# AllenInstitute/distributed-vae

Measured on AMD Instinct MI355X. Metric: cells/sec per train step (fwd+loss+bwd+opt), higher is better.
Workload: dtype f32; 1 GPU; cpl_mixVAE A=2 arms, synthetic-10x-v1 50000 cells x 5000 genes per GPU, batch 5000/GPU, fp32, H=100 L=10 C=92 S=2, x_drop=0.5, Adam lr=1e-3; global_batch=5000, parallelism=dp1, noise=in-kernel Philox4x32-10

## Files before the change

### distributed-vae_amd/_native.py

```python
from __future__ import annotations

import ctypes as C
import os
from typing import Dict, Optional

import torch

HERE = os.path.dirname(os.path.abspath(__file__))
LIB_PATH = os.environ.get("MMVAE_LIB") or os.path.join(HERE, "libmmvae_hip.so")

ABI_VERSION = 5
N_PARAM_TENSORS = 28
N_BN = 6
MAX_ARMS = 8

PARAM_NAMES = [
    "fc1.weight", "fc1.bias", "fc2.weight", "fc2.bias", "fc3.weight", "fc3.bias", "fc4.weight", "fc4.bias",
    "fc5.weight", "fc5.bias", "fcc.weight", "fcc.bias", "fc_mu.weight", "fc_sigma.weight", "fc_mu.bias",
    "fc_sigma.bias", "fc6.weight", "fc6.bias", "fc7.weight", "fc7.bias", "fc8.weight", "fc8.bias",
    "fc9.weight", "fc9.bias", "fc10.weight", "fc10.bias", "fc11.weight", "fc11.bias",
]
BN_NAMES = ["batch_l1", "batch_l2", "batch_l3", "batch_l4", "batch_l5", "batch_s"]

WS_IDS = {name: i for i, name in enumerate([
# ... 89 lines not shown
    out = (C.c_int32 * PLAN_FIELDS)()
    check(lib().mmvae_debug_plan(C.byref(dims), C.byref(hyper), C.byref(ex) if ex is not None else None, CALL_KINDS[kind],
                                 int(params_align), int(x_align), int(x_arm_stride), int(bool(has_x16)), int(bool(fc11_grad)),
                                 C.byref(out)), "mmvae_debug_plan")
    plan = {}
    for name, v in zip(PLAN_NAMES, out):
        if name in PLAN_ENUMS:
            plan[name] = PLAN_ENUMS[name][v]
        elif name == "kind":
            plan[name] = next(k for k, i in CALL_KINDS.items() if i == v)
        elif name in ("gd10_slabs", "dw11_slabs"):
            plan[name] = int(v)
        else:
            plan[name] = bool(v)
    return plan


_lib = None


def lib():
    global _lib
    if _lib is not None:
        return _lib
    if not os.path.exists(LIB_PATH):
        raise NativeError(
            f"{LIB_PATH} not found: build the HIP extension first "
            "(python -c 'import __graft_entry__ as g; g.build()' or python distributed-vae_amd/build.py). "
            "There is no CPU fallback.")
    L = C.CDLL(LIB_PATH)
# ... 15 lines not shown
                                 C.c_size_t, vp, ex, vp]
    L.mmvae_adam_step.argtypes = [i64, vp, vp, vp, vp, i64, f32, f32, f32, f32, f32, i32, vp]
    L.mmvae_train_step.argtypes = [C.POINTER(Dims), C.POINTER(Hyper), C.POINTER(Noise), vp, vp, vp, vp, i64, vp,
                                   C.c_size_t, vp, vp, i32, vp, vp, i64, f32, f32, f32, f32, f32, i32, ex, vp]
    L.mmvae_train_step_rows.argtypes = [C.POINTER(Dims), C.POINTER(Hyper), C.POINTER(Noise), vp, vp, vp, vp, vp, i64, i64, vp, vp,
                                        C.c_size_t, vp, vp, i32, vp, vp, i64, f32, f32, f32, f32, f32, i32, ex, vp]
    L.mmvae_train_step_rows.restype = C.c_int
    L.mmvae_to_bf16.argtypes = [vp, i64, i64, i32, vp, vp]
    L.mmvae_to_bf16.restype = C.c_int
    L.mmvae_debug_stage.argtypes = [C.POINTER(Dims), C.POINTER(Hyper), C.POINTER(Noise), i32, vp, vp, i64, vp,
                                    C.c_size_t, vp, ex, vp]
    L.mmvae_dump_noise.argtypes = [C.POINTER(Dims), C.POINTER(Hyper), C.POINTER(Noise), vp, vp, vp, vp, vp]
    L.mmvae_debug_plan.argtypes = [C.POINTER(Dims), C.POINTER(Hyper), ex, i32, i32, i32, i64, i32, i32,
                                   C.POINTER(C.c_int32 * PLAN_FIELDS)]
    L.mmvae_debug_plan.restype = C.c_int
    L.mmvae_eval_classify.argtypes = [C.POINTER(Dims), C.POINTER(Hyper), vp, vp, vp, i64, vp, C.c_size_t, vp, vp, ex,
                                      vp]
    L.mmvae_classify.argtypes = [vp, i64, i32, vp, vp]
    L.mmvae_confmat_accumulate.argtypes = [vp, i32, i64, i32, vp, vp]
    L.mmvae_consensus.argtypes = [vp, i32, i32, vp, vp, vp]
    L.mmvae_aug_packed_floats.argtypes = [C.POINTER(AugDims)]
    L.mmvae_aug_packed_floats.restype = C.c_size_t
    L.mmvae_aug_workspace_bytes.argtypes = [C.POINTER(AugDims), i32]
    L.mmvae_aug_workspace_bytes.restype = C.c_size_t
    L.mmvae_aug_pack.argtypes = [C.POINTER(AugDims), C.POINTER(AugTensors), vp, vp]
    L.mmvae_augment.argtypes = [C.POINTER(AugDims), vp, vp, i64, vp, vp, f32, vp, C.c_size_t, vp, vp, i32, ex, vp]
    L.mmvae_gather_rows.argtypes = [vp, i64, i64, vp, i64, i32, vp, vp]
    L.mmvae_tp_planes_bytes.argtypes = [i64, i32, i32]
    L.mmvae_tp_planes_bytes.restype = C.c_size_t
    L.mmvae_tp_planes.argtypes = [vp, i64, i64, i32, i32, vp, vp]
# ... 338 lines not shown
```

### distributed-vae_amd/csrc/api.hip

```cpp
#include "common.hpp"
#include <stdarg.h>
#include <stdio.h>
#include <string.h>

namespace mmvae {

static thread_local char g_err[512] = "";
void set_error(const char* fmt, ...) {
    va_list ap;
    va_start(ap, fmt);
    vsnprintf(g_err, sizeof(g_err), fmt, ap);
    va_end(ap);
}

Splits default_splits(const mmvae_dims& d, const mmvae_exec* ex) {
    int g_split[6] = {0, 0, 0, 0, 0, 0};
    if (ex) for (int i = 0; i < 6; ++i) g_split[i] = ex->split[i] > 0 && ex->split[i] <= 64 ? ex->split[i] : 0;
    constexpr int CUS = 256;
    auto fit = [](int base_blocks, int slots, int cap) {
        const int base = base_blocks > 0 ? base_blocks : 1;
        auto eff = [&](int k) { const int n = base * k; return (double)n / (double)(((n + slots - 1) / slots) * slots); };
        int pick = 1;
        double best = 0.0;
        for (int k = 1; k <= cap; ++k) {
            if (eff(k) >= 0.93) { pick = k; break; }
            if (eff(k) > best + 1e-9) { best = eff(k); pick = k; }
        }
        for (int k = pick + 1; k <= cap && k <= pick + 2; ++k)
            if (eff(k) >= 0.995) return k;
// ... 35 lines not shown
        if (g_split[5] <= 0) {
            const int nwg = max(1, pairs_d * d.A);
            const bool chain_x3 = chain_planes_fit(d) && !ex->tune[MMVAE_TUNE_CHAIN_FP32];
            const int target = chain_x3 ? 140 : 3 * CUS / 8;
            s.ks_dw11 = min(max(1, (target + nwg / 2) / nwg), max(1, cdiv(d.B, 32)));
        }
        if (g_split[3] <= 0) s.ks_small = min(fit(cdiv(N_SMALL * d.A, 2), CUS, 32), max(1, cdiv(d.B, 32)));
    }
    if (ex && ex->tune[MMVAE_TUNE_ENGINE] == 1 && fastdims && bf16_tiles_fit(d)) {
        if (g_split[3] <= 0) s.ks_small = min(fit(cdiv(N_SMALL * d.A, 2), CUS, 32), max(1, cdiv(d.B, 32)));
        if (g_split[5] <= 0) {
            const int nwg = max(1, cdiv(d.D, 128) * d.A);
            s.ks_dw11 = min(max(1, (5 * CUS / 8 + nwg / 2) / nwg), max(1, cdiv(d.B, 32)));
        }
    }
    return s;
}

POff make_poff(const mmvae_dims& d) {
    POff p{};
    const int64_t D = d.D, H = d.H, L = d.L, C = d.C, S = d.S;
    const int64_t sizes[MMVAE_N_PARAM_TENSORS] = {
        H * D, H, H * H, H, H * H, H, H * H, H, L * H, L, C * L, C, S * (L + C), S * (L + C), S, S,
        L * (C + S), L, H * L, H, H * H, H, H * H, H, H * H, H, D * H, D};
    int64_t off = 0;
    for (int t = 0; t < MMVAE_N_PARAM_TENSORS; ++t) {
        if (t != 13 && t != 15) off = cdiv64(off, 4) * 4;
        p.o[t] = off;
        off += sizes[t];
    }
// ... 41 lines not shown
    L.acc_end = off;
    L.GD10_slab = take((int64_t)max(L.sp.ns_fc11, L.sp.ks_gd10) * A * B * H);
    L.DZ11 = take(A * B * D);
    L.couple_part = take(nb * 2);
    L.T_part = take(nb * A * C); L.T = take(A * C);
    for (int i = 1; i <= 10; ++i) L.DZ[i] = take(A * B * ((i == 5 || i == 6) ? Ld : H));
    L.GZIN = take(A * B * (C + S)); L.GMS = take(A * B * 2 * S); L.GZC = take(A * B * C);
    for (int i = 1; i <= 5; ++i) {
        const int64_t W = (i == 5) ? Ld : H;
        L.G[i] = take(A * B * W);
        L.bnb_part[i] = take(A * (i == 5 ? (nb > cdiv(B, LAT_ROWS_BWD) ? nb : (int64_t)cdiv(B, LAT_ROWS_BWD)) : nb) * 2 * W);
        L.bnb_sum[i] = take(A * 2 * W);
    }
    L.dw1_slab = take((int64_t)L.sp.ks_dw * A * H * D);
    L.dw11_slab = take((int64_t)max(L.sp.ks_dw, L.sp.ks_dw11) * A * D * DW11_LD);
    L.small_slab = take((int64_t)L.sp.ks_small * A * N_SMALL * NP * SMALL_LD);
    L.xbits = take(A * B * cdiv(d.D, 32));
    {
        const int64_t Dk = cdiv64(D, 32) * 32, Dr = cdiv64(D, 128) * 128, Br = cdiv64(B, 256) * 256;
        L.pl_w1 = take(A * 3 * 128 * Dk / 2);
        L.pl_w11 = take(A * 3 * Dr * 128 / 2);
        L.pl_dz1 = take(A * 3 * Br * 128 / 2);
        L.pl_d10 = take(A * 3 * Br * 128 / 2);
        L.pl_small = take(A * (int64_t)PL_SMALL_SLOTS * 3 * 128 * 128 / 2);
    }
    L.rowmap = take(B + MAP_PAD);
    L.total = off;
    return L;
}

static int check_dims(const mmvae_dims* d) {
// ... 95 lines not shown
    else if (fc11_grad && d.H == 100 && (int64_t)cdiv(d.B, 256) * L.sp.ks_gd10 <= L.n11) p.fc11 = FC11_ZG;
    else p.fc11 = FC11_ZT;
    p.gd10_slabs = p.fast ? L.sp.ks_gd10 : L.sp.ns_fc11;
    p.dw11_slabs = p.fast ? L.sp.ks_dw11 : L.sp.ks_dw;
    p.chain_planes = p.fast && bf16_tiles && chain_planes_fit(d) && !c.tune(MMVAE_TUNE_CHAIN_FP32);
    p.lat_half = d.C <= 32 * LH_CPL && d.L <= 32 && 2 * d.S <= 32;
    p.narrow = h.gemm_bf16 == 1 && c.x16 != nullptr && bf16_tiles_fit(d) && (d.D & 7) == 0;
    p.presplit = fwd && p.fast && (x3 || p.chain_planes);
    p.bwd_small_planes = kind == CALL_BACKWARD && p.chain_planes;
    p.d10_planes = x3;
    p.dz1_in_apply = (x3 || p.narrow) && (d.H & 1) == 0;
    if (fwd && h.training) p.zero = p.presplit && dropout ? ZERO_PRESPLIT : p.fast && dropout ? ZERO_XBITS : ZERO_MEMSET;
    p.rowmap = kind == CALL_STEP_ROWS && p.zero == ZERO_PRESPLIT && slots && (p.fc11 == FC11_X3 || p.fc11 == FC11_BF16);
    p.dz11_bf16 = p.rowmap && c.x16 != nullptr && p.fc11 == FC11_BF16;
    p.dw11_side = (step || kind == CALL_BACKWARD) && p.fast && side;
    p.loss_on_side = step && p.fast && side;
    const int cs = c.tune(MMVAE_TUNE_COUPLE_SIDE);
    const bool role = p.loss_on_side && c.use_acc() && p.chain_planes && d.A >= 2 && d.A <= 5 && cs != 1 && (d.A >= 4 || cs == 3);
    p.couple = step && side ? (role ? COUPLE_IN_DEC : COUPLE_SIDE) : COUPLE_INLINE;
    p.lat_fork_rides = p.couple == COUPLE_SIDE && p.lat_half;
    p.fc11_fork_rides = p.loss_on_side && (p.fc11 == FC11_X3 || p.fc11 == FC11_BF16);
    if (kind == CALL_DECODE) {
        if (!p.fast) p.fc11 = FC11_GENERAL;
        else if (p.big == GEMM_X3 && x3_fc11_fits(d)) p.fc11 = FC11_OUT_X3;
        else if (p.big == GEMM_BF16) p.fc11 = FC11_OUT_BF16;
        else p.fc11 = FC11_ZT;
        p.d10_planes = p.fc11 == FC11_OUT_X3 || p.fc11 == FC11_OUT_BF16;
        p.dec_planes = p.d10_planes || p.chain_planes;
    }
}
// ... 95 lines not shown
static int do_loss(const Ctx& c, float* loss_out) {
    int rc;
    if ((rc = launch_couple(c))) return rc;
    return launch_loss_finalize(c, loss_out);
}

static int do_backward(const Ctx& c, const mmvae_noise* nz, const float* params, const float* x, int64_t xs,
                       float grad_scale, float* grads, const AdamHost* adam = nullptr, float* loss_out = nullptr) {
    const Plan& p = c.plan;
    int rc;
    const bool early = p.dw11_side && !adam && c.ex.early_grad_event != nullptr;
    const bool side_red = p.dw11_side && adam;
    if (c.ex_out) c.ex_out->early_recorded = 0;
    Ctx cs = c;
    cs.stream = c.side();
    if (p.dw11_side) {
        if ((rc = fork_to_side(c, EV_FORK, p.fc11_fork_rides))) return rc;
        if ((rc = dw11(cs))) return rc;
        if (early) {
            if ((rc = launch_reduce_grads(cs, grads, grad_scale, nullptr, 1))) return rc;
            if (hipEventRecord(reinterpret_cast<hipEvent_t>(c.ex.early_grad_event), c.side()) != hipSuccess) {
                set_error("event record failed");
                return MMVAE_E_LAUNCH;
            }
            if (c.ex_out) c.ex_out->early_recorded = 1;
        }
        if (side_red) {
            if ((rc = launch_reduce_grads(cs, grads, grad_scale, adam, 1))) return rc;
        }
        if (p.loss_on_side && (rc = launch_loss_finalize(cs, loss_out, 2))) return rc;
        if ((rc = record_on_side(c, EV_JOIN))) return rc;
    }
    if (p.bwd_small_planes && (rc = launch_x3_planes(c, params, false))) return rc;
    if ((rc = launch_chain_bwd_dec(c, params))) return rc;
    if (p.loss_on_side && p.couple == COUPLE_SIDE && (rc = join_from_side(c, EV_COUPLE))) return rc;
    if ((rc = launch_lat_bwd(c, nz, params))) return rc;
    for (int layer = 5; layer >= 2; --layer)
        if ((rc = launch_chain_bwd_enc(c, layer, params))) return rc;
    if ((rc = launch_bn_bwd_apply1(c))) return rc;
    if (p.big == GEMM_GENERAL) {
        if ((rc = launch_dw_big(c, nz, x, xs))) return rc;
    } else {
        if ((rc = dw1(c, x, xs))) return rc;
        if (!p.dw11_side && (rc = dw11(c))) return rc;
    }
    if ((rc = launch_dw_small(c))) return rc;
    if (p.dw11_side && (rc = join_from_side(c, EV_JOIN))) return rc;
    return launch_reduce_grads(c, grads, grad_scale, adam, early || side_red ? 2 : 3);
}

}

using namespace mmvae;

extern "C" {

int mmvae_abi_version(void) { return 5; }
const char* mmvae_last_error_string(void) { return g_err; }
int mmvae_check_dims(const mmvae_dims* d) { return check_dims(d); }

int mmvae_param_layout(const mmvae_dims* d, mmvae_param_layout_t* out) {
// ... 310 lines not shown
            if (stage == 10) return fc11_main(c, params, x, x_arm_stride, nullptr, 1);
            if (stage == 11) return fc11_gd10(c, params, nullptr, 1);
            if (stage == 12) return dw1(c, x, x_arm_stride);
            if (stage == 13) return dw11(c);
            return fc1_gemm(c, params, x, x_arm_stride);
        case 3: return launch_dw_small(c);
        case 4: return launch_chain_fwd_dec(c, params);
        case 5: return launch_chain_bwd_dec(c, params);
        case 6: return launch_lat_fwd(c, nz, params, nullptr, nullptr);
        case 7: return launch_lat_bwd(c, nz, params);
        case 8: if (!grads) { set_error("grads is null"); return MMVAE_E_BADARG; } return launch_reduce_grads(c, grads, 1.f, nullptr);
        default: set_error("unknown stage %d", stage); return MMVAE_E_BADARG;
    }
}

int mmvae_debug_plan(const mmvae_dims* d, const mmvae_hyper* h, const mmvae_exec* ex, int call_kind, int params_align,
                     int x_align, int64_t x_arm_stride, int has_x16, int fc11_grad, int32_t out[MMVAE_PLAN_FIELDS]) {
    if (int rc = check_dims(d)) return rc;
    if (!h || !out) { set_error("null hyper / out"); return MMVAE_E_BADARG; }
    if (int rc = check_gemm_engine(h->gemm_bf16)) return rc;
    static_assert(MMVAE_CALL_STEP == CALL_STEP && MMVAE_CALL_STEP_ROWS == CALL_STEP_ROWS && MMVAE_CALL_FORWARD == CALL_FORWARD &&
                  MMVAE_CALL_BACKWARD == CALL_BACKWARD && MMVAE_CALL_LOSS == CALL_LOSS && MMVAE_CALL_CLASSIFY == CALL_CLASSIFY &&
                  MMVAE_CALL_REPLAY == CALL_REPLAY && MMVAE_CALL_DECODE == CALL_DECODE && MMVAE_CALL_TRAVERSE == CALL_TRAVERSE,
                  "MMVAE_CALL_* (include/mmvae.h) are the values of CallKind");
    if (call_kind < CALL_STEP || call_kind > CALL_TRAVERSE) { set_error("unknown call kind %d", call_kind); return MMVAE_E_BADARG; }
    if (params_align < 0 || x_align < 0) { set_error("negative alignment"); return MMVAE_E_BADARG; }
    Ctx c{};
    c.d = *d;
    c.h = *h;
    if (call_kind == CALL_DECODE || call_kind == CALL_TRAVERSE || call_kind == CALL_CLASSIFY) c.h.training = 0;
    if (ex) c.ex = *ex; else memset(&c.ex, 0, sizeof(c.ex));
    c.lay = make_layout(*d, &c.ex);
    c.po = make_poff(*d);
    const uintptr_t base = 1u << 20;
    const float* params = reinterpret_cast<const float*>(base + (uintptr_t)(params_align & 15));
    const float* x = reinterpret_cast<const float*>(2 * base + (uintptr_t)(x_align & 15));
    if (has_x16 && call_kind == CALL_STEP_ROWS) c.x16 = reinterpret_cast<const unsigned short*>(3 * base);
    make_plan(c, (CallKind)call_kind, params, x, x_arm_stride, fc11_grad != 0);
    const Plan& p = c.plan;
    const int32_t v[] = {(int32_t)p.kind, p.fast, (int32_t)p.big, p.small_x3, (int32_t)p.fc11, p.gd10_slabs, p.dw11_slabs, p.chain_planes,
                         p.lat_half, p.narrow, p.presplit, p.bwd_small_planes, p.d10_planes, p.dz1_in_apply, p.dec_planes,
                         (int32_t)p.zero, p.rowmap, p.dz11_bf16, p.dw11_side, p.loss_on_side, (int32_t)p.couple, p.lat_fork_rides,
                         p.fc11_fork_rides};
    static_assert(sizeof(v) / sizeof(v[0]) == MMVAE_PLAN_FIELDS, "one value per field of Plan, in declaration order");
    for (int i = 0; i < MMVAE_PLAN_FIELDS; ++i) out[i] = v[i];
    return 0;
}

int mmvae_dump_noise(const mmvae_dims* d, const mmvae_hyper* h, const mmvae_noise* nz, uint8_t* x_mask,
                     float* u_gumbel, float* u_state, uint8_t* s_mask, void* stream) {
    if (int rc = check_dims(d)) return rc;
    if (!h || !nz) { set_error("null hyper / noise"); return MMVAE_E_BADARG; }
    return launch_dump_noise(*d, *h, nz, x_mask, u_gumbel, u_state, s_mask, reinterpret_cast<hipStream_t>(stream));
}

}
```

### distributed-vae_amd/csrc/common.hpp

```cpp
#pragma once
#include <hip/hip_runtime.h>
#include <hip/hip_ext.h>
#include <stdint.h>
#include "../../include/mmvae.h"
#include "tune.h"

namespace mmvae {

typedef float f32x16 __attribute__((ext_vector_type(16)));

constexpr int WAVE = 64;
constexpr int ROWS32 = 32;
constexpr int NP = 128;
constexpr int MAP_PAD = 256;
constexpr int DW11_LD = 132;
constexpr int SMALL_LD = 256;

__host__ __device__ inline int cdiv(int a, int b) { return (a + b - 1) / b; }
__host__ __device__ inline int64_t cdiv64(int64_t a, int64_t b) { return (a + b - 1) / b; }
__host__ __device__ inline int rup(int a, int b) { return cdiv(a, b) * b; }
__host__ __device__ inline int64_t imin64(int64_t a, int64_t b) { return a < b ? a : b; }

struct Splits {
    int ks_fc1;
    int ns_fc11;
    int ks_dw;
    int ks_dw11;
    int ks_small;
    int ks_gd10;
};

constexpr int N_SMALL = 12;

struct Layout {
    int nblk32;
    int nblk64;
    Splits sp;
    int64_t R[5];
    int nblkc;
    int chain_rows_fwd, nblkf;
    int nblkl;
    int64_t bn_mean[5], bn_rstd[5];
    int64_t bn_part[5];
    int64_t XLOW, CPROB, CC, YSOFT, CSMP, Y, MS, MU, LV, SS, ZIN;
    int64_t Dk[5];
    int64_t c_part, c_mean, c_iv;
    int64_t lat_part;
    int64_t fc1_slab;
    int n11;
    int64_t fc11_part;
    int64_t GD10_slab;
    int64_t DZ11;
    int64_t couple_part;
    int64_t T_part, T;
    int64_t DZ[11];
    int64_t GZIN, GMS, GZC, G[6];
    int64_t bnb_part[6], bnb_sum[6];
    int64_t dw1_slab;
    int64_t dw11_slab;
    int64_t small_slab;
    int64_t xbits;
    int64_t pl_w1;
    int64_t pl_w11;
    int64_t pl_dz1;
    int64_t pl_d10;
    int64_t pl_small;
    int64_t acc;
    int64_t acc_end;
    int64_t rowmap;
    int64_t total;
};
constexpr int PL_SMALL_LAYERS = 9, PL_SMALL_DEC0 = 4, PL_SMALL_SLOTS = 2 * PL_SMALL_LAYERS;
constexpr int ACC_W = 128;
constexpr int ACC_SET_I64 = 6 * ACC_W + 8;
constexpr int ACC_SET_FLOATS = 2 * ACC_SET_I64;
// ... 530 lines not shown
                const u32x4 r = xmask_words(nz, arm, (uint32_t)row, (uint32_t)(w * ncall + j));
                for (int e = 0; e < epc; ++e) word |= xmask_field_keep(nz, r, (uint32_t)e) ? (1u << (j * epc + e)) : 0u;
            }
            const int left = D - 32 * w;
            if (left < 32) word &= (1u << left) - 1u;
            out[w] = word;
        }
    }
}
#endif

inline bool fast_dims(const mmvae_dims& d) { return (d.D & 3) == 0 && (d.H & 3) == 0; }
inline bool bf16_tiles_fit(const mmvae_dims& d) { return d.H <= 124; }
inline bool x3_fc11_fits(const mmvae_dims& d) { return d.H + 1 <= 112; }
inline bool chain_planes_fit(const mmvae_dims& d) { return d.C + d.S <= 128 && d.L <= 128; }
inline bool fc11_slots_fit(const Layout& L, int B) { return (int64_t)cdiv(B, 128) * L.sp.ks_gd10 <= L.n11; }

enum CallKind { CALL_STEP, CALL_STEP_ROWS, CALL_FORWARD, CALL_BACKWARD, CALL_LOSS, CALL_CLASSIFY, CALL_REPLAY ,
                CALL_DECODE , CALL_TRAVERSE  };
enum GemmFamily { GEMM_GENERAL, GEMM_FP32, GEMM_BF16, GEMM_X3 };
enum Fc11Family { FC11_GENERAL, FC11_ZG, FC11_ZT, FC11_BF16, FC11_X3, FC11_OUT_BF16, FC11_OUT_X3 };
enum FwdZero { ZERO_NONE, ZERO_MEMSET, ZERO_XBITS , ZERO_PRESPLIT  };
enum CouplePlace { COUPLE_INLINE, COUPLE_SIDE, COUPLE_IN_DEC };
struct Plan {
    CallKind kind;
    bool fast;
    GemmFamily big;
    bool small_x3;
    Fc11Family fc11;
    int gd10_slabs;
// ... 2 lines not shown
    bool lat_half;
    bool narrow;
    bool presplit;
    bool bwd_small_planes;
    bool d10_planes;
    bool dz1_in_apply;
    bool dec_planes;
    FwdZero zero;
    bool rowmap;
    bool dz11_bf16;
    bool dw11_side;
    bool loss_on_side;
    CouplePlace couple;
    bool lat_fork_rides;
    bool fc11_fork_rides;
};

struct Ctx {
    mmvae_dims d;
    mmvae_hyper h;
    Layout lay;
    POff po;
    float* ws;
    hipStream_t stream;
    mmvae_exec ex;
    mmvae_exec* ex_out;
    hipStream_t side() const { return reinterpret_cast<hipStream_t>(ex.side_stream); }
    hipEvent_t ev(int i) const { return reinterpret_cast<hipEvent_t>(ex.ev[i]); }
    int tune(int i) const { return ex.tune[i]; }
    bool use_acc() const { return !ex.tune[MMVAE_TUNE_BN_PARTIALS]; }
// ... 7 lines not shown
    Plan plan{};
};
inline int zero_fc11_part(const Ctx& c) {
    if (c.plan.zero != ZERO_NONE) return 0;
    hipError_t e = hipMemsetAsync(c.ws + c.lay.fc11_part, 0, sizeof(float) * 2 * (size_t)c.d.A * c.lay.n11, c.stream);
    if (e != hipSuccess) { set_error("memset: %s", hipGetErrorString(e)); return MMVAE_E_LAUNCH; }
    return 0;
}
#ifdef __HIPCC__
template <class K, class... Args>
inline void launch_k(const Ctx& c, hipEvent_t stop_ev, K kernel, dim3 grid, dim3 block, unsigned shm, Args... args) {
    if (stop_ev) hipExtLaunchKernelGGL(kernel, grid, block, shm, c.stream, nullptr, stop_ev, 0, args...);
    else hipLaunchKernelGGL(kernel, grid, block, shm, c.stream, args...);
}
#endif
enum { EV_LAT = 0, EV_COUPLE, EV_FC11, EV_FORK, EV_JOIN, EV_DEC, EV_ENC, EV_SPARE  };

#ifdef __HIPCC__
NoiseDev make_noise_dev(const mmvae_noise* nz, const mmvae_hyper& h);
#endif

int launch_fc1_fwd(const Ctx& c, const mmvae_noise* nz, const float* params, const float* x, int64_t xs);
int launch_bn_eval_stats(const Ctx& c, const float* bn_running);
int launch_chain_fwd_enc(const Ctx& c, int layer , const float* params, float* bn_running, int64_t* nbt);
int launch_chain_fwd_enc_eval(const Ctx& c, const float* params);
int launch_lat_fwd(const Ctx& c, const mmvae_noise* nz, const float* params, float* bn_running, int64_t* nbt,
                   int32_t* labels = nullptr );
int launch_chain_fwd_dec(const Ctx& c, const float* params);
int launch_fc11_fused(const Ctx& c, const float* params, const float* x, int64_t xs, float* x_rec, int need_grad);
int launch_couple(const Ctx& c);
int launch_loss_finalize(const Ctx& c, float* loss_out, int mode = 0 );
// ... 2 lines not shown
int launch_chain_bwd_enc(const Ctx& c, int layer , const float* params);
int launch_bn_bwd_apply1(const Ctx& c);
int launch_dw_big(const Ctx& c, const mmvae_noise* nz, const float* x, int64_t xs);
int launch_dw_small(const Ctx& c, int which = 3 );
struct TnDesc {
    const float* P; int64_t p_arm_stride; int ldp; int Mv;
    const float* Q; int64_t q_arm_stride; int ldq; int Nv;
    int q_ones;
    int q_xmask;
    const float* q_mean;
    const float* q_rstd;
    float* out; int64_t out_arm_stride; int64_t out_ks_stride; int ldo;
};

struct TnDescs { TnDesc d[N_SMALL]; };
int launch_dw_small_x3(const Ctx& c, const TnDescs& ts, int nsel);
struct AdamHost { float* p; float* m; float* v; int64_t step; float lr, b1, b2, eps, wd; int decoupled; };
int launch_reduce_grads(const Ctx& c, float* grads, float grad_scale, const AdamHost* adam,
                        int which = 3 );
int launch_adam(int64_t n, float* p, const float* g, float* m, float* v, int64_t step, float lr, float b1,
                float b2, float eps, float wd, int decoupled, hipStream_t s);
int launch_make_xbits(const Ctx& c, const mmvae_noise* nz);
int launch_forward_zero(const Ctx& c, const mmvae_noise* nz);
int launch_fc1_epi(const Ctx& c, const float* params);
int launch_fc1_fwd_fp32(const Ctx& c, const float* params, const float* x, int64_t xs);
int launch_fc11_zg(const Ctx& c, const float* params, const float* x, int64_t xs, float* x_rec, int need_grad);
int launch_fc11_zt(const Ctx& c, const float* params, const float* x, int64_t xs, float* x_rec, int need_grad);
int launch_gd10_fp32(const Ctx& c, const float* params);
int launch_dw1_fp32(const Ctx& c, const float* x, int64_t xs);
int launch_dw11_fp32(const Ctx& c);
int launch_x3_planes(const Ctx& c, const float* params, bool head, const mmvae_noise* nz = nullptr);
// ... 44 lines not shown
```

### distributed-vae_amd/csrc/gemm_bf16.hip

```cpp
#include "common.hpp"

namespace mmvae {

typedef __bf16 bf16x8 __attribute__((ext_vector_type(8)));
typedef __bf16 bf16x2 __attribute__((ext_vector_type(2)));
typedef unsigned int u32x4v __attribute__((ext_vector_type(4)));


constexpr int BT = 128;
constexpr int KT = 64;
constexpr int LDB = 36;
constexpr int LDK = 136;

template <int NP>
struct Eng {
    static constexpr int KT = NP == 1 ? 64 : 32;
    static constexpr int NQ = KT / 8;
    static constexpr int LDB = KT / 2 + 4;
    static constexpr int PLANE = BT * LDB;
    static constexpr int LDK = NP == 1 ? 136 : 160;
    static constexpr int NBUF = NP == 1 ? 2 : 1;
};

__device__ __forceinline__ unsigned pack_bf16(float a, float b) {
// ... 1689 lines not shown

int launch_dw11_bf16(const Ctx& c) {
    const mmvae_dims& d = c.d;
    const Layout& L = c.lay;
    GemmArgs g{};
    g.a = kminor(c.ws + L.DZ11, d.D, d.D, d.B); g.a_arm = (int64_t)d.B * d.D;
    g.b = kminor(c.ws + L.Dk[4], d.H, d.H, d.B); g.b_arm = (int64_t)d.B * d.H;
    g.b.ones_row = d.H;
    if (c.plan.big == GEMM_X3) use_planes(c, g.b, PL_D10);
    else if (c.plan.dz11_bf16) { g.a.src16 = 1; g.a_arm /= 2; }
    g.M = d.D; g.N = d.H + 1; g.K = d.B; g.KS = L.sp.ks_dw11; g.A = d.A;
    g.so = SlabOut{c.ws + L.dw11_slab, (int64_t)d.A * d.D * DW11_LD, (int64_t)d.D * DW11_LD, DW11_LD, d.D, d.H + 1};
    return launch_slab_gemm(c, g, 2, slab_grid(c, g, d.D), "k_bf16_gemm<dW11>");
}

int launch_dw_small_x3(const Ctx& c, const TnDescs& ts, int nsel) {
    const int KS = c.lay.sp.ks_small;
    hipLaunchKernelGGL(k_x3_small, dim3(cdiv(nsel * c.d.A, 2), KS), dim3(512), 0, c.stream, ts, nsel, c.d.A, c.d.B, KS);
    HIP_LAUNCH_CHECK("k_x3_small");
    return 0;
}

}
```

### distributed-vae_amd/csrc/gemm_big.hip

```cpp
#include "common.hpp"

namespace mmvae {

__device__ __forceinline__ float4 load_x4(const float* __restrict__ x, int row, int col, int B, int D,
                                          bool vec_ok) {
    float4 v = make_float4(0.f, 0.f, 0.f, 0.f);
    if (row < B) {
        const float* p = x + (int64_t)row * D + col;
        if (vec_ok && col + 3 < D) {
            v = *reinterpret_cast<const float4*>(p);
        } else {
            if (col < D) v.x = p[0];
            if (col + 1 < D) v.y = p[1];
            if (col + 2 < D) v.z = p[2];
            if (col + 3 < D) v.w = p[3];
        }
    }
    return v;
}

__device__ __forceinline__ float4 apply_xmask(float4 v, const NoiseDev& nz, int use_mask, int arm, int row,
                                              int col, int B, int D, bool vec_ok) {
    if (!use_mask || row >= B || col >= D) return v;
    const int64_t idx = ((int64_t)arm * B + row) * D + col;
// ... 615 lines not shown
        hipLaunchKernelGGL((k_gemm_tn<128, 64>), grid, dim3(256), 0, c.stream, t1, 1, nd, d.B, KS, 1 | (vx ? 2 : 0));
        HIP_LAUNCH_CHECK("k_gemm_tn<dW1>");
    }
    {
        dim3 grid(cdiv(d.D, 64) * cdiv(d.H + 1, 128), KS, d.A);
        hipLaunchKernelGGL((k_gemm_tn<64, 128>), grid, dim3(256), 0, c.stream, t2, 1, nd, d.B, KS, 3);
        HIP_LAUNCH_CHECK("k_gemm_tn<dW11>");
    }
    return 0;
}

int launch_dw_small(const Ctx& c, int which) {
    const mmvae_dims& d = c.d;
    const Layout& L = c.lay;
    const int A = d.A, B = d.B, H = d.H, Ld = d.L, C = d.C, S = d.S;
    const int KS = L.sp.ks_small;
    TnDescs ts{}, all{};
    TnDesc* hd = all.d;
    NoiseDev nd{};
    const int64_t slab_ks = (int64_t)A * N_SMALL * NP * SMALL_LD;
    auto mk = [&](int i, int64_t dz, int N, int64_t xin, int K, int64_t mean, int64_t rstd) {
        hd[i] = TnDesc{c.ws + dz, (int64_t)B * N, N, N, c.ws + xin, (int64_t)B * K, K, K, 1, 0,
                       mean >= 0 ? c.ws + mean : nullptr, rstd >= 0 ? c.ws + rstd : nullptr,
                       c.ws + L.small_slab + (int64_t)i * NP * SMALL_LD, (int64_t)N_SMALL * NP * SMALL_LD, slab_ks,
                       SMALL_LD};
    };
    mk(0, L.DZ[2], H, L.R[0], H, L.bn_mean[0], L.bn_rstd[0]);
    mk(1, L.DZ[3], H, L.R[1], H, L.bn_mean[1], L.bn_rstd[1]);
    mk(2, L.DZ[4], H, L.R[2], H, L.bn_mean[2], L.bn_rstd[2]);
    mk(3, L.DZ[5], Ld, L.R[3], H, L.bn_mean[3], L.bn_rstd[3]);
    mk(4, L.GZC, C, L.XLOW, Ld, -1, -1);
    mk(5, L.GMS, 2 * S, L.Y, Ld + C, -1, -1);
    mk(6, L.DZ[6], Ld, L.ZIN, C + S, -1, -1);
    mk(7, L.DZ[7], H, L.Dk[0], Ld, -1, -1);
    mk(8, L.DZ[8], H, L.Dk[1], H, -1, -1);
    mk(9, L.DZ[9], H, L.Dk[2], H, -1, -1);
    mk(10, L.DZ[10], H, L.Dk[3], H, -1, -1);
    mk(11, L.DZ[1], H, L.R[0], 0, -1, -1);
    int nsel = 0, tiles = 1;
    for (int i = 0; i < N_SMALL; ++i) {
        const bool dec = i >= 6 && i <= 10;
        if (!(which & (dec ? 1 : 2))) continue;
        ts.d[nsel++] = hd[i];
        tiles = max(tiles, cdiv(hd[i].Mv, 128) * cdiv(hd[i].Nv + 1, 128));
    }
    if (nsel == 0) return 0;
    if (c.plan.small_x3) {
        bool fits = true;
        for (int i = 0; i < nsel; ++i) fits = fits && ts.d[i].Mv <= 128 && ts.d[i].Nv + ts.d[i].q_ones <= 128 && !ts.d[i].q_xmask;
        if (fits) return launch_dw_small_x3(c, ts, nsel);
    }
    dim3 grid(tiles, KS, A * nsel);
    hipLaunchKernelGGL((k_gemm_tn<128, 128>), grid, dim3(256), 0, c.stream, ts, nsel, nd, B, KS, 3);
    HIP_LAUNCH_CHECK("k_gemm_tn<small>");
    return 0;
}

}
```

### distributed-vae_amd/csrc/rowwise.hip

```cpp
#include "common.hpp"
#include "couple.hpp"
#include <type_traits>
#include <math.h>
#include <stdlib.h>

namespace mmvae {


NoiseDev make_noise_dev(const mmvae_noise* nz, const mmvae_hyper& h) {
    NoiseDev n{};
    n.mode = nz ? nz->mode : 0;
    if (nz) {
        n.x_mask = nz->x_mask; n.u_gumbel = nz->u_gumbel; n.u_state = nz->u_state; n.s_mask = nz->s_mask;
        n.k0 = (uint32_t)nz->seed; n.k1 = (uint32_t)(nz->seed >> 32);
        n.step_lo = (uint32_t)nz->offset; n.step_hi = (uint32_t)(nz->offset >> 32);
    }
    const uint32_t t16 = keep_threshold16(h.x_drop);
    uint32_t ml = 0;
    while (ml < 4 && (t16 & ((65536u >> (1u << ml)) - 1u)) != 0) ++ml;
    n.x_mlog2 = ml;
    n.x_thr = t16 >> (16u - (1u << ml));
    n.s_keep_thr = keep_threshold(h.s_drop);
    return n;
}
// ... 911 lines not shown
        if (mode == 1) return 0;
        mode = 2;
    }
    const int nT = cdiv(d.A * d.C, 32);
    hipLaunchKernelGGL(k_loss_finalize, dim3(mode == 0 ? 1 + nT : (mode == 1 ? nT : 1)), dim3(256), 0, c.stream, d.A, d.B, d.D, d.C,
                       c.h.beta, c.h.lam, c.ws + L.fc11_part, L.n11, c.ws + L.lat_part, L.nblkl, L.nblk32, c.ws + L.couple_part,
                       c.ws + L.T_part, c.ws + L.T, loss_out, mode);
    HIP_LAUNCH_CHECK("k_loss_finalize");
    return 0;
}

int launch_lat_bwd(const Ctx& c, const mmvae_noise* nz, const float* params) {
    LatArgs a = make_lat_args(c);
    NoiseDev nd = make_noise_dev(nz, c.h);
    const size_t shm = lat_smem_bytes(c.d);
    if (c.plan.lat_half) {
        hipLaunchKernelGGL(k_lat_bwd_h, dim3(cdiv(c.d.B, LAT_ROWS_BWD), c.d.A), dim3(64 * LBH_NW), shm, c.stream, a, nd, params, c.ws);
        HIP_LAUNCH_CHECK("k_lat_bwd_h");
        return 0;
    }
    hipLaunchKernelGGL(k_lat_bwd, dim3(cdiv(c.d.B, LAT_ROWS_BWD), c.d.A), dim3(64 * LATB_NW), shm, c.stream, a, nd, params, c.ws);
    HIP_LAUNCH_CHECK("k_lat_bwd");
    return 0;
}

int launch_reduce_grads(const Ctx& c, float* grads, float gscale, const AdamHost* ah, int which) {
    const mmvae_dims& d = c.d;
    const Layout& L = c.lay;
    const int A = d.A, H = d.H, D = d.D, Ld = d.L, C = d.C, S = d.S;
    RedDescs ds{};
    int n = 0;
    const float xscale = c.dropout() ? 1.f / (1.f - c.h.x_drop) : 1.f;
    const int ks11 = c.plan.dw11_slabs;
    ds.d[n++] = RedDesc{c.ws + L.dw1_slab, (int64_t)A * H * D, (int64_t)H * D, D, 0, H, D, c.po.o[0], D, gscale * xscale, L.sp.ks_dw};
    ds.d[n++] = RedDesc{c.ws + L.dw11_slab, (int64_t)A * D * DW11_LD, (int64_t)D * DW11_LD, DW11_LD, 0, D, H, c.po.o[26], H, gscale, ks11};
    ds.d[n++] = RedDesc{c.ws + L.dw11_slab, (int64_t)A * D * DW11_LD, (int64_t)D * DW11_LD, DW11_LD, H, D, 1, c.po.o[27], 1, gscale, ks11};
    const int nbig = n;
    const int64_t sks = (int64_t)A * N_SMALL * NP * SMALL_LD, sarm = (int64_t)N_SMALL * NP * SMALL_LD;
    auto small = [&](int i, int N, int K, int64_t w_off, int64_t b_off) {
        const float* s = c.ws + L.small_slab + (int64_t)i * NP * SMALL_LD;
        if (K > 0) ds.d[n++] = RedDesc{s, sks, sarm, SMALL_LD, 0, N, K, w_off, K, gscale, L.sp.ks_small};
        ds.d[n++] = RedDesc{s, sks, sarm, SMALL_LD, K, N, 1, b_off, 1, gscale, L.sp.ks_small};
    };
    small(0, H, H, c.po.o[2], c.po.o[3]);
    small(1, H, H, c.po.o[4], c.po.o[5]);
    small(2, H, H, c.po.o[6], c.po.o[7]);
    small(3, Ld, H, c.po.o[8], c.po.o[9]);
    small(4, C, Ld, c.po.o[10], c.po.o[11]);
    small(5, 2 * S, Ld + C, c.po.o[12], c.po.o[14]);
    small(6, Ld, C + S, c.po.o[16], c.po.o[17]);
    small(7, H, Ld, c.po.o[18], c.po.o[19]);
    small(8, H, H, c.po.o[20], c.po.o[21]);
    small(9, H, H, c.po.o[22], c.po.o[23]);
    small(10, H, H, c.po.o[24], c.po.o[25]);
    small(11, H, 0, 0, c.po.o[1]);
    AdamArgs aa{};
    if (ah && ah->p) {
// ... 88 lines not shown
```

### include/mmvae.h

```cpp
#ifndef MMVAE_H
#define MMVAE_H

#include <stddef.h>
#include <stdint.h>

#ifdef __cplusplus
extern "C" {
#endif

#define MMVAE_OK 0
#define MMVAE_E_BADARG (-1)
#define MMVAE_E_UNSUPPORTED (-2)
#define MMVAE_E_LAUNCH (-3)
#define MMVAE_E_WORKSPACE (-4)

#define MMVAE_MAX_ARMS 8
#define MMVAE_N_PARAM_TENSORS 28
#define MMVAE_N_BN 6

typedef struct mmvae_dims {
    int32_t A, B, D, H, L, C, S;
} mmvae_dims;

typedef struct mmvae_hyper {
// ... 185 lines not shown
                      size_t ws_bytes, float *grads, mmvae_exec *ex, void *stream);

#define MMVAE_PLAN_FIELDS 23
#define MMVAE_CALL_STEP 0
#define MMVAE_CALL_STEP_ROWS 1
#define MMVAE_CALL_FORWARD 2
#define MMVAE_CALL_BACKWARD 3
#define MMVAE_CALL_LOSS 4
#define MMVAE_CALL_CLASSIFY 5
#define MMVAE_CALL_REPLAY 6
#define MMVAE_CALL_DECODE 7
#define MMVAE_CALL_TRAVERSE 8
int mmvae_debug_plan(const mmvae_dims *d, const mmvae_hyper *h, const mmvae_exec *ex, int call_kind,
                     int params_align, int x_align, int64_t x_arm_stride, int has_x16, int fc11_grad,
                     int32_t out[MMVAE_PLAN_FIELDS]);

#ifdef __cplusplus
}
#endif
#endif
```

Measured before the change: 7.332 million cells/s.

## Split small-layer weight grads into early/late groups, run early group on side stream

```diff
diff --git a/distributed-vae_amd/_native.py b/distributed-vae_amd/_native.py
--- a/distributed-vae_amd/_native.py
+++ b/distributed-vae_amd/_native.py
@@ -127,6 +127,18 @@
         else:
             plan[name] = bool(v)
     return plan
+
+
+PLAN_SMALL_NAMES = ("small_early_side", "small_ks_early", "small_ks_late", "ks_small", "ks_small_early", "ks_small_late")
+
+
+def debug_plan_small(dims: "Dims", hyper: "Hyper", ex: Optional["Exec"], kind: str, params_align: int = 16, x_align: int = 16,
+                     x_arm_stride: int = 0, has_x16: bool = False, fc11_grad: bool = True) -> Dict[str, object]:
+    out = (C.c_int32 * len(PLAN_SMALL_NAMES))()
+    check(lib().mmvae_debug_plan_small(C.byref(dims), C.byref(hyper), C.byref(ex) if ex is not None else None, CALL_KINDS[kind],
+                                       int(params_align), int(x_align), int(x_arm_stride), int(bool(has_x16)),
+                                       int(bool(fc11_grad)), C.byref(out)), "mmvae_debug_plan_small")
+    return {n: (bool(v) if n == "small_early_side" else int(v)) for n, v in zip(PLAN_SMALL_NAMES, out)}
 
 
 _lib = None
@@ -172,6 +184,9 @@
     L.mmvae_debug_plan.argtypes = [C.POINTER(Dims), C.POINTER(Hyper), ex, i32, i32, i32, i64, i32, i32,
                                    C.POINTER(C.c_int32 * PLAN_FIELDS)]
     L.mmvae_debug_plan.restype = C.c_int
+    L.mmvae_debug_plan_small.argtypes = [C.POINTER(Dims), C.POINTER(Hyper), ex, i32, i32, i32, i64, i32, i32,
+                                         C.POINTER(C.c_int32 * len(PLAN_SMALL_NAMES))]
+    L.mmvae_debug_plan_small.restype = C.c_int
     L.mmvae_eval_classify.argtypes = [C.POINTER(Dims), C.POINTER(Hyper), vp, vp, vp, i64, vp, C.c_size_t, vp, vp, ex,
                                       vp]
     L.mmvae_classify.argtypes = [vp, i64, i32, vp, vp]
diff --git a/distributed-vae_amd/csrc/api.hip b/distributed-vae_amd/csrc/api.hip
--- a/distributed-vae_amd/csrc/api.hip
+++ b/distributed-vae_amd/csrc/api.hip
@@ -13,6 +13,8 @@
     va_end(ap);
 }
 
+constexpr bool SMALL_TAIL_FIRST = false;
+constexpr int SMALL_EARLY_WG = 96;
 Splits default_splits(const mmvae_dims& d, const mmvae_exec* ex) {
     int g_split[6] = {0, 0, 0, 0, 0, 0};
     if (ex) for (int i = 0; i < 6; ++i) g_split[i] = ex->split[i] > 0 && ex->split[i] <= 64 ? ex->split[i] : 0;
@@ -78,6 +80,14 @@
             s.ks_dw11 = min(max(1, (5 * CUS / 8 + nwg / 2) / nwg), max(1, cdiv(d.B, 32)));
         }
     }
+    s.ks_small_early = s.ks_small_late = s.ks_small;
+    const int eng = ex ? ex->tune[MMVAE_TUNE_ENGINE] : 0;
+    if (ex && (eng == 1 || eng == 2) && fastdims && bf16_tiles_fit(d) && small_x3_fits(d) && g_split[3] <= 0) {
+        const int kmax = max(1, cdiv(d.B, 32));
+        const int nb_e = cdiv(N_SMALL_EARLY * d.A, 2), nb_l = cdiv(N_SMALL_LATE * d.A, 2);
+        s.ks_small_early = min(min(max(1, (SMALL_EARLY_WG + nb_e / 2) / nb_e), 64), kmax);
+        s.ks_small_late = min(fit(nb_l, CUS, 64), kmax);
+    }
     return s;
 }
 
@@ -149,7 +159,8 @@
     }
     L.dw1_slab = take((int64_t)L.sp.ks_dw * A * H * D);
     L.dw11_slab = take((int64_t)max(L.sp.ks_dw, L.sp.ks_dw11) * A * D * DW11_LD);
-    L.small_slab = take((int64_t)L.sp.ks_small * A * N_SMALL * NP * SMALL_LD);
+    L.small_slab_early = take((int64_t)max(L.sp.ks_small, L.sp.ks_small_early) * A * N_SMALL_EARLY * NP * SMALL_LD);
+    L.small_slab_late = take((int64_t)max(L.sp.ks_small, L.sp.ks_small_late) * A * N_SMALL_LATE * NP * SMALL_LD);
     L.xbits = take(A * B * cdiv(d.D, 32));
     {
         const int64_t Dk = cdiv64(D, 32) * 32, Dr = cdiv64(D, 128) * 128, Br = cdiv64(B, 256) * 256;
@@ -275,6 +286,9 @@
     p.rowmap = kind == CALL_STEP_ROWS && p.zero == ZERO_PRESPLIT && slots && (p.fc11 == FC11_X3 || p.fc11 == FC11_BF16);
     p.dz11_bf16 = p.rowmap && c.x16 != nullptr && p.fc11 == FC11_BF16;
     p.dw11_side = (step || kind == CALL_BACKWARD) && p.fast && side;
+    p.small_early_side = p.dw11_side && p.small_x3 && small_x3_fits(d);
+    p.small_ks_early = p.small_early_side ? L.sp.ks_small_early : L.sp.ks_small;
+    p.small_ks_late = p.small_early_side ? L.sp.ks_small_late : L.sp.ks_small;
     p.loss_on_side = step && p.fast && side;
     const int cs = c.tune(MMVAE_TUNE_COUPLE_SIDE);
     const bool role = p.loss_on_side && c.use_acc() && p.chain_planes && d.A >= 2 && d.A <= 5 && cs != 1 && (d.A >= 4 || cs == 3);
@@ -400,6 +414,12 @@
     if (c.ex_out) c.ex_out->early_recorded = 0;
     Ctx cs = c;
     cs.stream = c.side();
+    auto side_tail = [&]() -> int {
+        if (side_red && (rc = launch_reduce_grads(cs, grads, grad_scale, adam, 1))) return rc;
+        if (p.loss_on_side && (rc = launch_loss_finalize(cs, loss_out, 2))) return rc;
+        return 0;
+    };
+    const bool tail_first = !p.small_early_side || SMALL_TAIL_FIRST;
     if (p.dw11_side) {
         if ((rc = fork_to_side(c, EV_FORK, p.fc11_fork_rides))) return rc;
         if ((rc = dw11(cs))) return rc;
@@ -411,16 +431,19 @@
             }
             if (c.ex_out) c.ex_out->early_recorded = 1;
         }
-        if (side_red) {
-            if ((rc = launch_reduce_grads(cs, grads, grad_scale, adam, 1))) return rc;
-        }
-        if (p.loss_on_side && (rc = launch_loss_finalize(cs, loss_out, 2))) return rc;
-        if ((rc = record_on_side(c, EV_JOIN))) return rc;
+        if (tail_first && (rc = side_tail())) return rc;
+        if (!p.small_early_side && (rc = record_on_side(c, EV_JOIN))) return rc;
     }
     if (p.bwd_small_planes && (rc = launch_x3_planes(c, params, false))) return rc;
     if ((rc = launch_chain_bwd_dec(c, params))) return rc;
     if (p.loss_on_side && p.couple == COUPLE_SIDE && (rc = join_from_side(c, EV_COUPLE))) return rc;
     if ((rc = launch_lat_bwd(c, nz, params))) return rc;
+    if (p.small_early_side) {
+        if ((rc = fork_to_side(c, EV_SMALL, true))) return rc;
+        if ((rc = launch_dw_small(cs, 1))) return rc;
+        if (!tail_first && (rc = side_tail())) return rc;
+        if ((rc = record_on_side(c, EV_JOIN))) return rc;
+    }
     for (int layer = 5; layer >= 2; --layer)
         if ((rc = launch_chain_bwd_enc(c, layer, params))) return rc;
     if ((rc = launch_bn_bwd_apply1(c))) return rc;
@@ -430,7 +453,7 @@
         if ((rc = dw1(c, x, xs))) return rc;
         if (!p.dw11_side && (rc = dw11(c))) return rc;
     }
-    if ((rc = launch_dw_small(c))) return rc;
+    if ((rc = launch_dw_small(c, p.small_early_side ? 2 : 3))) return rc;
     if (p.dw11_side && (rc = join_from_side(c, EV_JOIN))) return rc;
     return launch_reduce_grads(c, grads, grad_scale, adam, early || side_red ? 2 : 3);
 }
@@ -771,8 +794,8 @@
     }
 }
 
-int mmvae_debug_plan(const mmvae_dims* d, const mmvae_hyper* h, const mmvae_exec* ex, int call_kind, int params_align,
-                     int x_align, int64_t x_arm_stride, int has_x16, int fc11_grad, int32_t out[MMVAE_PLAN_FIELDS]) {
+static int debug_make_plan(Ctx& c, const mmvae_dims* d, const mmvae_hyper* h, const mmvae_exec* ex, int call_kind, int params_align,
+                           int x_align, int64_t x_arm_stride, int has_x16, int fc11_grad, const void* out) {
     if (int rc = check_dims(d)) return rc;
     if (!h || !out) { set_error("null hyper / out"); return MMVAE_E_BADARG; }
     if (int rc = check_gemm_engine(h->gemm_bf16)) return rc;
@@ -782,7 +805,7 @@
                   "MMVAE_CALL_* (include/mmvae.h) are the values of CallKind");
     if (call_kind < CALL_STEP || call_kind > CALL_TRAVERSE) { set_error("unknown call kind %d", call_kind); return MMVAE_E_BADARG; }
     if (params_align < 0 || x_align < 0) { set_error("negative alignment"); return MMVAE_E_BADARG; }
-    Ctx c{};
+    c = Ctx{};
     c.d = *d;
     c.h = *h;
     if (call_kind == CALL_DECODE || call_kind == CALL_TRAVERSE || call_kind == CALL_CLASSIFY) c.h.training = 0;
@@ -794,6 +817,13 @@
     const float* x = reinterpret_cast<const float*>(2 * base + (uintptr_t)(x_align & 15));
     if (has_x16 && call_kind == CALL_STEP_ROWS) c.x16 = reinterpret_cast<const unsigned short*>(3 * base);
     make_plan(c, (CallKind)call_kind, params, x, x_arm_stride, fc11_grad != 0);
+    return 0;
+}
+
+int mmvae_debug_plan(const mmvae_dims* d, const mmvae_hyper* h, const mmvae_exec* ex, int call_kind, int params_align,
+                     int x_align, int64_t x_arm_stride, int has_x16, int fc11_grad, int32_t out[MMVAE_PLAN_FIELDS]) {
+    Ctx c;
+    if (int rc = debug_make_plan(c, d, h, ex, call_kind, params_align, x_align, x_arm_stride, has_x16, fc11_grad, out)) return rc;
     const Plan& p = c.plan;
     const int32_t v[] = {(int32_t)p.kind, p.fast, (int32_t)p.big, p.small_x3, (int32_t)p.fc11, p.gd10_slabs, p.dw11_slabs, p.chain_planes,
                          p.lat_half, p.narrow, p.presplit, p.bwd_small_planes, p.d10_planes, p.dz1_in_apply, p.dec_planes,
@@ -804,6 +834,18 @@
     return 0;
 }
 
+int mmvae_debug_plan_small(const mmvae_dims* d, const mmvae_hyper* h, const mmvae_exec* ex, int call_kind, int params_align,
+                           int x_align, int64_t x_arm_stride, int has_x16, int fc11_grad, int32_t out[MMVAE_PLAN_SMALL_FIELDS]) {
+    Ctx c;
+    if (int rc = debug_make_plan(c, d, h, ex, call_kind, params_align, x_align, x_arm_stride, has_x16, fc11_grad, out)) return rc;
+    const Plan& p = c.plan;
+    const Splits& sp = c.lay.sp;
+    const int32_t v[] = {p.small_early_side, p.small_ks_early, p.small_ks_late, sp.ks_small, sp.ks_small_early, sp.ks_small_late};
+    static_assert(sizeof(v) / sizeof(v[0]) == MMVAE_PLAN_SMALL_FIELDS, "one value per field");
+    for (int i = 0; i < MMVAE_PLAN_SMALL_FIELDS; ++i) out[i] = v[i];
+    return 0;
+}
+
 int mmvae_dump_noise(const mmvae_dims* d, const mmvae_hyper* h, const mmvae_noise* nz, uint8_t* x_mask,
                      float* u_gumbel, float* u_state, uint8_t* s_mask, void* stream) {
     if (int rc = check_dims(d)) return rc;
diff --git a/distributed-vae_amd/csrc/common.hpp b/distributed-vae_amd/csrc/common.hpp
--- a/distributed-vae_amd/csrc/common.hpp
+++ b/distributed-vae_amd/csrc/common.hpp
@@ -27,10 +27,15 @@
     int ks_dw;
     int ks_dw11;
     int ks_small;
+    int ks_small_early, ks_small_late;
     int ks_gd10;
 };
 
 constexpr int N_SMALL = 12;
+constexpr int SMALL_EARLY0 = 4, N_SMALL_EARLY = 7, N_SMALL_LATE = N_SMALL - N_SMALL_EARLY;
+inline bool small_is_early(int i) { return i >= SMALL_EARLY0 && i < SMALL_EARLY0 + N_SMALL_EARLY; }
+inline int small_slot(int i) { return small_is_early(i) ? i - SMALL_EARLY0 : i < SMALL_EARLY0 ? i : i - N_SMALL_EARLY; }
+inline int small_group_n(int i) { return small_is_early(i) ? N_SMALL_EARLY : N_SMALL_LATE; }
 
 struct Layout {
     int nblk32;
@@ -58,7 +63,7 @@
     int64_t bnb_part[6], bnb_sum[6];
     int64_t dw1_slab;
     int64_t dw11_slab;
-    int64_t small_slab;
+    int64_t small_slab_early, small_slab_late;
     int64_t xbits;
     int64_t pl_w1;
     int64_t pl_w11;
@@ -619,6 +624,9 @@
 inline bool bf16_tiles_fit(const mmvae_dims& d) { return d.H <= 124; }
 inline bool x3_fc11_fits(const mmvae_dims& d) { return d.H + 1 <= 112; }
 inline bool chain_planes_fit(const mmvae_dims& d) { return d.C + d.S <= 128 && d.L <= 128; }
+inline bool small_x3_fits(const mmvae_dims& d) {
+    return d.H + 1 <= 128 && d.L + d.C + 1 <= 128 && d.C + d.S + 1 <= 128 && d.C <= 128 && 2 * d.S <= 128 && d.L + 1 <= 128;
+}
 inline bool fc11_slots_fit(const Layout& L, int B) { return (int64_t)cdiv(B, 128) * L.sp.ks_gd10 <= L.n11; }
 
 enum CallKind { CALL_STEP, CALL_STEP_ROWS, CALL_FORWARD, CALL_BACKWARD, CALL_LOSS, CALL_CLASSIFY, CALL_REPLAY ,
@@ -651,6 +659,8 @@
     CouplePlace couple;
     bool lat_fork_rides;
     bool fc11_fork_rides;
+    bool small_early_side;
+    int small_ks_early, small_ks_late;
 };
 
 struct Ctx {
@@ -688,7 +698,7 @@
     else hipLaunchKernelGGL(kernel, grid, block, shm, c.stream, args...);
 }
 #endif
-enum { EV_LAT = 0, EV_COUPLE, EV_FC11, EV_FORK, EV_JOIN, EV_DEC, EV_ENC, EV_SPARE  };
+enum { EV_LAT = 0, EV_COUPLE, EV_FC11, EV_FORK, EV_JOIN, EV_DEC, EV_ENC, EV_SMALL  };
 
 #ifdef __HIPCC__
 NoiseDev make_noise_dev(const mmvae_noise* nz, const mmvae_hyper& h);
@@ -721,7 +731,7 @@
 };
 
 struct TnDescs { TnDesc d[N_SMALL]; };
-int launch_dw_small_x3(const Ctx& c, const TnDescs& ts, int nsel);
+int launch_dw_small_x3(const Ctx& c, const TnDescs& ts, int nsel, int KS);
 struct AdamHost { float* p; float* m; float* v; int64_t step; float lr, b1, b2, eps, wd; int decoupled; };
 int launch_reduce_grads(const Ctx& c, float* grads, float grad_scale, const AdamHost* adam,
                         int which = 3 );
diff --git a/distributed-vae_amd/csrc/gemm_bf16.hip b/distributed-vae_amd/csrc/gemm_bf16.hip
--- a/distributed-vae_amd/csrc/gemm_bf16.hip
+++ b/distributed-vae_amd/csrc/gemm_bf16.hip
@@ -1727,8 +1727,7 @@
     return launch_slab_gemm(c, g, 2, slab_grid(c, g, d.D), "k_bf16_gemm<dW11>");
 }
 
-int launch_dw_small_x3(const Ctx& c, const TnDescs& ts, int nsel) {
-    const int KS = c.lay.sp.ks_small;
+int launch_dw_small_x3(const Ctx& c, const TnDescs& ts, int nsel, int KS) {
     hipLaunchKernelGGL(k_x3_small, dim3(cdiv(nsel * c.d.A, 2), KS), dim3(512), 0, c.stream, ts, nsel, c.d.A, c.d.B, KS);
     HIP_LAUNCH_CHECK("k_x3_small");
     return 0;
diff --git a/distributed-vae_amd/csrc/gemm_big.hip b/distributed-vae_amd/csrc/gemm_big.hip
--- a/distributed-vae_amd/csrc/gemm_big.hip
+++ b/distributed-vae_amd/csrc/gemm_big.hip
@@ -653,16 +653,20 @@
     const mmvae_dims& d = c.d;
     const Layout& L = c.lay;
     const int A = d.A, B = d.B, H = d.H, Ld = d.L, C = d.C, S = d.S;
-    const int KS = L.sp.ks_small;
+    const int KS = which == 1 ? c.plan.small_ks_early : which == 2 ? c.plan.small_ks_late : L.sp.ks_small;
+    if (which == 3 && (c.plan.small_ks_early != KS || c.plan.small_ks_late != KS)) {
+        set_error("internal: one small-layer launch under a plan that sums %d / %d slabs", c.plan.small_ks_early, c.plan.small_ks_late);
+        return MMVAE_E_LAUNCH;
+    }
     TnDescs ts{}, all{};
     TnDesc* hd = all.d;
     NoiseDev nd{};
-    const int64_t slab_ks = (int64_t)A * N_SMALL * NP * SMALL_LD;
+    const int64_t prod = (int64_t)NP * SMALL_LD;
     auto mk = [&](int i, int64_t dz, int N, int64_t xin, int K, int64_t mean, int64_t rstd) {
         hd[i] = TnDesc{c.ws + dz, (int64_t)B * N, N, N, c.ws + xin, (int64_t)B * K, K, K, 1, 0,
                        mean >= 0 ? c.ws + mean : nullptr, rstd >= 0 ? c.ws + rstd : nullptr,
-                       c.ws + L.small_slab + (int64_t)i * NP * SMALL_LD, (int64_t)N_SMALL * NP * SMALL_LD, slab_ks,
-                       SMALL_LD};
+                       c.ws + (small_is_early(i) ? L.small_slab_early : L.small_slab_late) + small_slot(i) * prod,
+                       small_group_n(i) * prod, A * small_group_n(i) * prod, SMALL_LD};
     };
     mk(0, L.DZ[2], H, L.R[0], H, L.bn_mean[0], L.bn_rstd[0]);
     mk(1, L.DZ[3], H, L.R[1], H, L.bn_mean[1], L.bn_rstd[1]);
@@ -678,8 +682,7 @@
     mk(11, L.DZ[1], H, L.R[0], 0, -1, -1);
     int nsel = 0, tiles = 1;
     for (int i = 0; i < N_SMALL; ++i) {
-        const bool dec = i >= 6 && i <= 10;
-        if (!(which & (dec ? 1 : 2))) continue;
+        if (!(which & (small_is_early(i) ? 1 : 2))) continue;
         ts.d[nsel++] = hd[i];
         tiles = max(tiles, cdiv(hd[i].Mv, 128) * cdiv(hd[i].Nv + 1, 128));
     }
@@ -687,8 +690,9 @@
     if (c.plan.small_x3) {
         bool fits = true;
         for (int i = 0; i < nsel; ++i) fits = fits && ts.d[i].Mv <= 128 && ts.d[i].Nv + ts.d[i].q_ones <= 128 && !ts.d[i].q_xmask;
-        if (fits) return launch_dw_small_x3(c, ts, nsel);
-    }
+        if (fits) return launch_dw_small_x3(c, ts, nsel, KS);
+    }
+    if (which != 3) { set_error("internal: a small-layer group launch off k_x3_small"); return MMVAE_E_LAUNCH; }
     dim3 grid(tiles, KS, A * nsel);
     hipLaunchKernelGGL((k_gemm_tn<128, 128>), grid, dim3(256), 0, c.stream, ts, nsel, nd, B, KS, 3);
     HIP_LAUNCH_CHECK("k_gemm_tn<small>");
diff --git a/distributed-vae_amd/csrc/rowwise.hip b/distributed-vae_amd/csrc/rowwise.hip
--- a/distributed-vae_amd/csrc/rowwise.hip
+++ b/distributed-vae_amd/csrc/rowwise.hip
@@ -949,12 +949,13 @@
     LatArgs a = make_lat_args(c);
     NoiseDev nd = make_noise_dev(nz, c.h);
     const size_t shm = lat_smem_bytes(c.d);
+    const hipEvent_t ev = c.plan.small_early_side ? c.ev(EV_SMALL) : nullptr;
     if (c.plan.lat_half) {
-        hipLaunchKernelGGL(k_lat_bwd_h, dim3(cdiv(c.d.B, LAT_ROWS_BWD), c.d.A), dim3(64 * LBH_NW), shm, c.stream, a, nd, params, c.ws);
+        launch_k(c, ev, k_lat_bwd_h, dim3(cdiv(c.d.B, LAT_ROWS_BWD), c.d.A), dim3(64 * LBH_NW), shm, a, nd, params, c.ws);
         HIP_LAUNCH_CHECK("k_lat_bwd_h");
         return 0;
     }
-    hipLaunchKernelGGL(k_lat_bwd, dim3(cdiv(c.d.B, LAT_ROWS_BWD), c.d.A), dim3(64 * LATB_NW), shm, c.stream, a, nd, params, c.ws);
+    launch_k(c, ev, k_lat_bwd, dim3(cdiv(c.d.B, LAT_ROWS_BWD), c.d.A), dim3(64 * LATB_NW), shm, a, nd, params, c.ws);
     HIP_LAUNCH_CHECK("k_lat_bwd");
     return 0;
 }
@@ -971,11 +972,14 @@
     ds.d[n++] = RedDesc{c.ws + L.dw11_slab, (int64_t)A * D * DW11_LD, (int64_t)D * DW11_LD, DW11_LD, 0, D, H, c.po.o[26], H, gscale, ks11};
     ds.d[n++] = RedDesc{c.ws + L.dw11_slab, (int64_t)A * D * DW11_LD, (int64_t)D * DW11_LD, DW11_LD, H, D, 1, c.po.o[27], 1, gscale, ks11};
     const int nbig = n;
-    const int64_t sks = (int64_t)A * N_SMALL * NP * SMALL_LD, sarm = (int64_t)N_SMALL * NP * SMALL_LD;
+    const int64_t prod = (int64_t)NP * SMALL_LD;
     auto small = [&](int i, int N, int K, int64_t w_off, int64_t b_off) {
-        const float* s = c.ws + L.small_slab + (int64_t)i * NP * SMALL_LD;
-        if (K > 0) ds.d[n++] = RedDesc{s, sks, sarm, SMALL_LD, 0, N, K, w_off, K, gscale, L.sp.ks_small};
-        ds.d[n++] = RedDesc{s, sks, sarm, SMALL_LD, K, N, 1, b_off, 1, gscale, L.sp.ks_small};
+        const bool e = small_is_early(i);
+        const float* s = c.ws + (e ? L.small_slab_early : L.small_slab_late) + small_slot(i) * prod;
+        const int64_t sarm = small_group_n(i) * prod, sks = A * sarm;
+        const int ks = e ? c.plan.small_ks_early : c.plan.small_ks_late;
+        if (K > 0) ds.d[n++] = RedDesc{s, sks, sarm, SMALL_LD, 0, N, K, w_off, K, gscale, ks};
+        ds.d[n++] = RedDesc{s, sks, sarm, SMALL_LD, K, N, 1, b_off, 1, gscale, ks};
     };
     small(0, H, H, c.po.o[2], c.po.o[3]);
     small(1, H, H, c.po.o[4], c.po.o[5]);
diff --git a/include/mmvae.h b/include/mmvae.h
--- a/include/mmvae.h
+++ b/include/mmvae.h
@@ -223,6 +223,10 @@
 int mmvae_debug_plan(const mmvae_dims *d, const mmvae_hyper *h, const mmvae_exec *ex, int call_kind,
                      int params_align, int x_align, int64_t x_arm_stride, int has_x16, int fc11_grad,
                      int32_t out[MMVAE_PLAN_FIELDS]);
+#define MMVAE_PLAN_SMALL_FIELDS 6
+int mmvae_debug_plan_small(const mmvae_dims *d, const mmvae_hyper *h, const mmvae_exec *ex, int call_kind,
+                           int params_align, int x_align, int64_t x_arm_stride, int has_x16, int fc11_grad,
+                           int32_t out[MMVAE_PLAN_SMALL_FIELDS]);
 
 #ifdef __cplusplus
 }
```

Result: slower. 7.220 million cells/s (-1.5%).
